# typio/entreepy

Measured on AMD Instinct MI355X. Metric: GB/s encode+decode on 1 GiB text at 1/2/4/8 MI355X; % of HBM read peak, higher is better.
Workload: dtype u8; 1 GPU; text-1G: 1073741824 B per GPU, order-0 samples of a_midsummer_nights_dream.txt's byte distribution, seed 0x5EED0004+rank, one step = encode to .et + decode back, HBM-resident; bytes_per_gpu=1073741824, packed_bytes_per_gpu=629699194

## Files before the change

entreepy_amd/codec.py:

```python
import ctypes
from dataclasses import dataclass

import numpy as np

from . import _native as N


class EntreepyError(RuntimeError):
    def __init__(self, status, detail=""):
        msg = N.lib().et_strerror(status).decode()
        super().__init__(f"{msg}{': ' + detail if detail else ''} (et_status {status})")
        self.status = status


class EmptyInputError(EntreepyError):
    """The reference's error.QueueEmpty (queue.zig:28-30 reached from encode.zig:137-138)."""


@dataclass
class EncodeFlags:
    write_output: bool = False
    print_output: bool = False
    debug: bool = False

# ... 150 lines not shown
        _check(N.lib().et_ctx_reserve(self._h, int(max_text_bytes)), self._h)

    def set_tile_rounds(self, rounds):
        _check(N.lib().et_ctx_set_tile_rounds(self._h, int(rounds)), self._h)

    TIMING_DECODE_BODY = 2

    def enable_timing(self, on=True):
        _check(N.lib().et_ctx_enable_timing(self._h, 2 if (on is not True and on == self.TIMING_DECODE_BODY) else int(bool(on))), self._h)

    def timings(self, which=None):
        t = N.Timings()
        if which is None:
            _check(N.lib().et_last_timings(self._h, ctypes.byref(t)), self._h)
        else:
            _check(N.lib().et_last_timings_of(self._h, {"encode": 0, "decode": 1}[which], ctypes.byref(t)), self._h)
        d = {k: getattr(t, k) for k, _ in N.Timings._fields_ if k not in ("reserved", "pad_")}
        d["exhaustive_sync"] = bool(t.reserved & 1)
        d["tree_walk_sync"] = bool(t.reserved & 2)
        d["chained_write"] = bool(t.reserved & 4)
        d["row_sync"] = bool(t.reserved & 8)
        d["fixed_sync"] = bool(t.reserved & 16)
        d["strips_write"] = bool(t.reserved & 32)
        return d

    def last_codebook(self):
        cb = Codebook()
        _check(N.lib().et_last_codebook(self._h, ctypes.byref(cb.raw)), self._h)
        return cb

    def encode_file(self, in_path, out_path=None):
        return self._file_call(N.lib().et_encode_fd, in_path, out_path, ())

    def decode_file(self, in_path, out_path=None, skip=4):
        return self._file_call(N.lib().et_decode_fd, in_path, out_path, (skip,))

    def _file_call(self, fn, in_path, out_path, extra):
        import os

        fin = os.open(in_path, os.O_RDONLY)
        fout = os.open(out_path, os.O_RDWR | os.O_CREAT | os.O_TRUNC, 0o644) if out_path is not None else -1
        try:
            a, b = ctypes.c_size_t(0), ctypes.c_size_t(0)
            _check(fn(self._h, fin, *extra, fout, ctypes.byref(a), ctypes.byref(b)), self._h)
            return a.value, b.value
        finally:
# ... 371 lines not shown
```

entreepy_amd/csrc/et_api.cpp:

```cpp
#include <sys/stat.h>

#include "et_ctx.h"

#include <algorithm>
#include <cstdlib>
#include <vector>

namespace {

struct Geometry {
    const uint8_t *base;
    uint64_t lo, hi;
    uint32_t rpt, n_tiles;
};

Geometry make_geometry(const et_ctx *ctx, const void *d_text, size_t n) {
    Geometry g;
    const uintptr_t a = reinterpret_cast<uintptr_t>(d_text);
    g.base = reinterpret_cast<const uint8_t *>(a & ~static_cast<uintptr_t>(15));
    g.lo = a & 15;
    g.hi = g.lo + n;
    uint32_t rpt = 1;
    while (rpt < et::MAX_ROUNDS_PER_TILE && g.hi / (static_cast<uint64_t>(rpt) * et::ROUND_BYTES) > 2048) rpt <<= 1;
    if (ctx && ctx->force_rpt) rpt = ctx->force_rpt;
// ... 34 lines not shown
    ctx->hist_tiles = g.n_tiles;
    ctx->hist_on_host = false;
    return ET_OK;
}

int run_body(et_ctx *ctx, const et_codebook *cb, const Geometry &g, uint32_t *out32, uint64_t base_bit,
             const uint8_t *header, size_t header_len, int ev_scan, int ev_body) {
    const bool long_codes = cb->max_length > 32;
    ET_TRY(wait_for_word<uint64_t>(ctx, ctx->h_scalar + HS_ENC_TAKEN, ctx->enc_block_epoch, 100.0, "the code table block was never taken"));
    for (int s = 0; s < 256; ++s) {
        const uint32_t len = cb->length[s];
        uint32_t code = cb->data[s];
        if (!long_codes) code = len ? (len == 32 ? code : (code & ((1u << len) - 1u)) << (32 - len)) : 0u;
        ctx->h_enc[2 * s] = code;
        ctx->h_enc[2 * s + 1] = len;
        ctx->h_enc[512 + s] = len;
    }
    const size_t padded = (header_len + 3) & ~static_cast<size_t>(3);
    if (header_len) {
        if (padded > HEADER_STAGE) return fail(ctx, ET_ERR_ARG, "header too long");
        uint8_t *stage = reinterpret_cast<uint8_t *>(ctx->h_enc + 768);
        std::memcpy(stage, header, header_len);
        std::memset(stage + header_len, 0, padded - header_len);
    }
    et::launch_tile_scan(ctx->stream, static_cast<const uint32_t *>(ctx->tile_hist.p), g.n_tiles, cb->length, ctx->h_enc, static_cast<uint32_t *>(ctx->enc_table.p),
                         static_cast<uint32_t>(768 + padded / 4), reinterpret_cast<unsigned long long *>(ctx->h_scalar + HS_ENC_TAKEN), ++ctx->enc_block_epoch,
                         static_cast<unsigned long long *>(ctx->tile_bits.p),
                         static_cast<unsigned long long *>(ctx->group_sum.p), scan_epoch(ctx), base_bit,
                         static_cast<unsigned long long *>(ctx->tile_off.p), out32, static_cast<const uint32_t *>(ctx->enc_table.p) + 768,
                         static_cast<uint32_t>(padded / 4));
    ET_HIP(hipGetLastError());
    et::launch_encode(ctx->stream, g.base, g.lo, g.hi, g.rpt, g.n_tiles, static_cast<const unsigned long long *>(ctx->tile_off.p),
                      static_cast<const uint2 *>(ctx->enc_table.p), cb->max_length, out32, timed(ctx, ev_scan, ev_body));
    ET_HIP(hipGetLastError());
    return ET_OK;
}

int fetch_histogram(et_ctx *ctx) {
    if (ctx->hist_on_host) return ET_OK;
    for (uint32_t w = 0; w < et::HIST_REDUCE_GROUPS; ++w)
        ET_TRY(wait_for_word<uint64_t>(ctx, ctx->h_hist + 256 + w, ctx->hist_epoch, 100.0, "the histogram never reached the host"));
    ctx->hist_on_host = true;
    return ET_OK;
}

}
// ... 24 lines not shown
    ok = ok && hipHostMalloc(reinterpret_cast<void **>(&ctx->h_enc), 768 * sizeof(uint32_t) + HEADER_STAGE) == hipSuccess;
    ok = ok && hipHostMalloc(reinterpret_cast<void **>(&ctx->h_header), HEADER_STAGE) == hipSuccess;
    for (int i = 0; i < 2; ++i) ok = ok && hipHostMalloc(reinterpret_cast<void **>(&ctx->h_lut_buf[i]), DEC_TABLES_BYTES) == hipSuccess;
    ok = ok && hipHostMalloc(reinterpret_cast<void **>(&ctx->h_scalar), HS_SLOTS * sizeof(uint64_t)) == hipSuccess;
    if (ok) std::memset(ctx->h_scalar, 0, HS_SLOTS * sizeof(uint64_t));
    for (int i = 0; i < 2; ++i) ok = ok && hipHostMalloc(reinterpret_cast<void **>(&ctx->h_tw_tree[i]), sizeof(et::TwUpload)) == hipSuccess;
    for (auto &e : ctx->ev) ok = ok && hipEventCreateWithFlags(&e, hipEventDisableSystemFence) == hipSuccess;
    if (!ok) {
        et_ctx_destroy(ctx);
        return ET_ERR_HIP;
    }
    *out = ctx;
    return ET_OK;
}

extern "C" void et_ctx_destroy(et_ctx *ctx) {
    if (!ctx) return;
    DeviceGuard guard(ctx->device);
    (void)hipStreamSynchronize(ctx->stream);
    DevBuf *bufs[] = {&ctx->tile_hist, &ctx->block_hist, &ctx->hist, &ctx->tile_bits, &ctx->tile_off, &ctx->enc_table, &ctx->group_sum,
                      &ctx->sub_state, &ctx->blk_exit, &ctx->blk_count, &ctx->blk_off, &ctx->lut, &ctx->flag,
                      &ctx->worklist, &ctx->lane_maps, &ctx->blk_maps, &ctx->grp_maps, &ctx->blk_in, &ctx->grp_in, &ctx->row_scratch,
                      &ctx->tw_table, &ctx->tw_tree, &ctx->blk_start, &ctx->blk_pub, &ctx->chain_table, &ctx->io_in, &ctx->io_out,
                      &ctx->batch_jobs, &ctx->batch_blob, &ctx->batch_counter};
    for (DevBuf *b : bufs)
        if (b->p) (void)hipFree(b->p);
    delete ctx->io;
    void *pinned[] = {ctx->h_hist, ctx->h_enc, ctx->h_header, ctx->h_lut_buf[0], ctx->h_lut_buf[1], ctx->h_scalar, ctx->h_tw_tree[0], ctx->h_tw_tree[1], ctx->h_batch};
    for (void *p : pinned)
        if (p) (void)hipHostFree(p);
    for (auto &e : ctx->ev)
        if (e) (void)hipEventDestroy(e);
    if (ctx->own_stream) (void)hipStreamDestroy(ctx->own_stream);
    if (ctx->side.stream) (void)hipStreamDestroy(ctx->side.stream);
    if (ctx->side.fork) (void)hipEventDestroy(ctx->side.fork);
    if (ctx->side.join) (void)hipEventDestroy(ctx->side.join);
    if (ctx->switch_ev) (void)hipEventDestroy(ctx->switch_ev);
    delete ctx;
}

namespace {

int switch_stream(et_ctx *ctx, hipStream_t s) {
    if (s == ctx->stream) return ET_OK;
    DeviceGuard guard(ctx->device);
    ET_HIP(hipEventRecord(ctx->switch_ev, ctx->stream));
    ET_HIP(hipStreamWaitEvent(s, ctx->switch_ev, 0));
// ... 40 lines not shown
        ET_HIP(hipEventSynchronize(ctx->ev[3]));
        if (!ctx->pend_enc_shard) {
            ctx->tm_enc.hist_ms = elapsed(ctx, 0, 1);
            ctx->tm_enc.total_ms = elapsed(ctx, 0, 3);
        }
        ctx->tm_enc.scan_ms = ctx->pend_enc_bits ? elapsed(ctx, 1, 2) : 0.f;
        ctx->tm_enc.body_ms = elapsed(ctx, 2, 3);
        ctx->pend_enc = ctx->pend_enc_shard = false;
    }
    if (which == 1 && ctx->pend_dec && ctx->timing_body) {
        ET_HIP(hipEventSynchronize(ctx->ev[EV_DEC + 3]));
        ctx->tm_dec.body_ms = elapsed(ctx, EV_DEC + 2, EV_DEC + 3);
        ctx->pend_dec = false;
    }
    if (which == 1 && ctx->pend_dec) {
        ET_HIP(hipEventSynchronize(ctx->ev[EV_DEC + 3]));
        ctx->tm_dec.sync_ms = elapsed(ctx, EV_DEC + 0, EV_DEC + 2);
        ctx->tm_dec.scan_ms = elapsed(ctx, EV_DEC + 5, EV_DEC + 2);
        ctx->tm_dec.body_ms = elapsed(ctx, EV_DEC + 2, EV_DEC + 3);
        ctx->tm_dec.total_ms = elapsed(ctx, EV_DEC + 0, EV_DEC + 3);
        ctx->tm_dec.sync_first_ms = ctx->pend_dec_first ? elapsed(ctx, EV_DEC + 0, EV_DEC + 5) : 0.f;
        ctx->pend_dec = false;
    }
    *out = which == 0 ? ctx->tm_enc : ctx->tm_dec;
    return ET_OK;
}

extern "C" int et_last_timings(et_ctx *ctx, et_timings *out) {
    if (!ctx) return ET_ERR_ARG;
    return et_last_timings_of(ctx, ctx->last_kind, out);
}

extern "C" int et_last_codebook(const et_ctx *ctx, et_codebook *out) {
    if (!ctx || !out) return ET_ERR_ARG;
    if (!ctx->have_cb) return ET_ERR_ARG;
    *out = ctx->last_cb;
    return ET_OK;
}

extern "C" int et_ctx_reserve(et_ctx *ctx, size_t max_text_bytes) {
    if (!ctx) return ET_ERR_ARG;
    DeviceGuard guard(ctx->device);
    const Geometry g = make_geometry(nullptr, reinterpret_cast<const void *>(static_cast<uintptr_t>(15)), max_text_bytes);
    ET_TRY(ensure_encode_ws(ctx, g.n_tiles + 1));
    const uint64_t n_subs = (static_cast<uint64_t>(max_text_bytes) + 8192) * 8 / et::SUB_BITS + 2;
    const uint64_t n_blocks = n_subs / et::BLOCK + 2;
// ... 25 lines not shown
        return ET_OK;
    }
    ctx->hist_empty = false;
    const Geometry g = make_geometry(ctx, d_text, n);
    ET_TRY(run_histogram(ctx, d_text, n, g, d_hist));
    if (ctx->timing) {
        ET_HIP(hipStreamSynchronize(ctx->stream));
        ctx->tm_enc = et_timings{};
        ctx->tm_enc.hist_ms = elapsed(ctx, 0, 1);
        ctx->pend_enc = false;
        ctx->last_kind = 0;
    }
    return ET_OK;
}

namespace {

int encode_shard(et_ctx *ctx, const et_codebook *cb, const void *d_text, size_t n, void *d_out, size_t cap_bytes, uint64_t start_bit,
                 const uint8_t *header, size_t header_len, uint64_t *end_bit) {
    if (!ctx || !cb || !d_out || !end_bit || (n && !d_text)) return ET_ERR_ARG;
    if (reinterpret_cast<uintptr_t>(d_out) & 3) return fail(ctx, ET_ERR_ARG, "d_out must be 4-byte aligned");
    if (header_len > HEADER_STAGE - 4) return fail(ctx, ET_ERR_ARG, "header too long");
    DeviceGuard guard(ctx->device);
    auto empty_shard = [&]() -> int {
        const size_t head_words = (header_len + 3) / 4;
        const size_t own_word = header_len ? 0 : static_cast<size_t>(start_bit / 32);
        const size_t need = (header_len ? head_words : own_word + 1) * 4;
        if (need > cap_bytes) return fail(ctx, ET_ERR_CAP, "body does not fit d_out");
        if (header_len) {
            std::memset(ctx->h_header, 0, head_words * 4);
            std::memcpy(ctx->h_header, header, header_len);
            ET_HIP(hipMemcpyAsync(d_out, ctx->h_header, head_words * 4, hipMemcpyHostToDevice, ctx->stream));
        } else {
            ET_HIP(hipMemsetAsync(static_cast<uint8_t *>(d_out) + own_word * 4, 0, 4, ctx->stream));
        }
        *end_bit = start_bit;
        return ET_OK;
    };
    if (n == 0) {
        ET_HIP(hipStreamSynchronize(ctx->stream));
        return empty_shard();
    }
    if (ctx->hist_text != d_text || ctx->hist_n != n)
        return fail(ctx, ET_ERR_ARG, "shard encode needs et_histogram_device on the same (d_text, n) first");
    ET_TRY(fetch_histogram(ctx));
    ET_HIP(hipStreamSynchronize(ctx->stream));
// ... 48 lines not shown
    std::memcpy(ctx->h_hist, counts, 256 * sizeof(uint64_t));
    ctx->hist_on_host = true;
    return ET_OK;
}

extern "C" int et_encode_body_device(et_ctx *ctx, const et_codebook *cb, const void *d_text, size_t n, void *d_out, size_t cap_bytes,
                                     uint64_t start_bit, uint64_t *end_bit) {
    return encode_shard(ctx, cb, d_text, n, d_out, cap_bytes, start_bit, nullptr, 0, end_bit);
}

extern "C" int et_encode_head_shard_device(et_ctx *ctx, const et_codebook *cb, const void *d_text, size_t n, void *d_out, size_t cap_bytes,
                                           const uint8_t *header, size_t header_len, uint64_t *end_bit) {
    if (!header || !header_len) return ET_ERR_ARG;
    return encode_shard(ctx, cb, d_text, n, d_out, cap_bytes, static_cast<uint64_t>(header_len) * 8, header, header_len, end_bit);
}

extern "C" int et_encode_device(et_ctx *ctx, const void *d_text, size_t n, void *d_out, size_t cap, size_t *out_len) {
    if (!ctx || !d_out || !out_len || (n && !d_text)) return ET_ERR_ARG;
    *out_len = 0;
    if (n == 0) return fail(ctx, ET_ERR_EMPTY, "empty input");
    if (reinterpret_cast<uintptr_t>(d_out) & 15) return fail(ctx, ET_ERR_ARG, "d_out must be 16-byte aligned");
    if (cap < et_encode_bound(n)) return fail(ctx, ET_ERR_CAP, "cap < et_encode_bound(n)");
    DeviceGuard guard(ctx->device);
    const Geometry g = make_geometry(ctx, d_text, n);
    ET_TRY(run_histogram(ctx, d_text, n, g));
    ET_TRY(fetch_histogram(ctx));
    const double t1 = now_ms();

    et_codebook cb;
    int rc = et_build_codebook(ctx->h_hist, &cb);
    if (rc != ET_OK) return fail(ctx, rc, "et_build_codebook");
    ctx->last_cb = cb;
    ctx->have_cb = true;
    size_t header_len = 0;
    std::memset(ctx->h_header, 0, HEADER_STAGE);
    rc = et_write_header(&cb, n, ctx->h_header, HEADER_STAGE - 4, &header_len);
    if (rc != ET_OK) return fail(ctx, rc, "et_write_header");
    uint64_t bits = 0;
    et_codebook_bits(&cb, ctx->h_hist, &bits);
    const double t2 = now_ms();

    if (bits == 0) {
        const size_t padded = (header_len + 3) & ~static_cast<size_t>(3);
        ET_HIP(hipMemcpyAsync(d_out, ctx->h_header, padded, hipMemcpyHostToDevice, ctx->stream));
        record(ctx, 2);
        record(ctx, 3);
// ... 167 lines not shown
```

entreepy_amd/csrc/et_ctx.h:

```cpp
#pragma once

#include "entreepy_hip.h"

#include "et_io.h"
#include "et_kernels.h"
#include "et_rowsync.h"
#include "et_tables.h"
#include "et_treewalk.h"

#include <hip/hip_runtime.h>

#include <atomic>
#include <chrono>
#include <cstdio>
#include <cstring>
#include <string>

struct DevBuf {
    void *p = nullptr;
    size_t cap = 0;
};

constexpr size_t HEADER_STAGE = 8192;
constexpr size_t DEC_TABLES_BYTES = et::DecTableLayout::BYTES;

enum class Family { TREE_WALK, WINDOWS, ROWS, FIXED_SYNC, FIXED_WRITE, EXIT_MAPS };

using et::DecWs;

struct Span : et::DecSpan {
    uint32_t tw_mode, dec_flags, row_mode;
    const et_codebook *cb;
    et::RowCode row_code;
    et::DecodeTables tb, tb_write;
    const uint16_t *tw_table;
    uint32_t tw_n_int;
    uint32_t *blk_start, *blk_pub;
    uint32_t *exit_bits;
    const uint64_t *chain;
    uint32_t n_chain;
};

enum HostScalar {
    HS_TOTAL = 1,
    HS_RANGE_FLAGS = 2,
    HS_BODY_FLAGS = 4,
    HS_ENC_TAKEN = 12,
    HS_HEADER_DONE = 14,
    HS_SLOTS = 16
};
enum RangeFlag { RF_START = 0, RF_EXIT = 1, RF_ROW_BLIND = 2 };

struct et_ctx {
    int device = 0;
    hipStream_t own_stream = nullptr;
    et::SideLane side = {};
    hipStream_t stream = nullptr;
    hipEvent_t switch_ev = nullptr;
    bool timing = false;
    bool timing_body = false;
    uint32_t force_rpt = 0;
    std::string err;

    DevBuf tile_hist, block_hist, hist, tile_bits, tile_off, enc_table, group_sum;
    DevBuf sub_state, blk_exit, blk_count, blk_off, lut, flag, worklist;
    DevBuf lane_maps, blk_maps, grp_maps, blk_in, grp_in;
    DevBuf row_scratch;
    DevBuf tw_table, tw_tree, blk_start, blk_pub, chain_table;
    et::TwUpload *h_tw_tree[2] = {};
    int tw_turn = 0;
    DevBuf io_in, io_out;
    et_io::Pipe *io = nullptr;

    DevBuf batch_jobs, batch_blob, batch_counter;
    uint8_t *h_batch = nullptr;
    uint64_t batch_epoch = 0;

    uint64_t *h_hist = nullptr;
    uint32_t *h_enc = nullptr;
    uint8_t *h_header = nullptr;
    uint8_t *h_lut_buf[2] = {};
    int lut_turn = 0;
    uint64_t *h_scalar = nullptr;

    const void *hist_text = nullptr;
    size_t hist_n = 0;
    uint32_t hist_rpt = 0, hist_tiles = 0;
// ... 68 lines not shown
        b.p = nullptr;
        return fail(ctx, e == hipErrorOutOfMemory ? ET_ERR_NOMEM : ET_ERR_HIP, "hipMalloc", e);
    }
    b.cap = want;
    return ET_OK;
}

#define ET_TRY(expr)                 \
    do {                             \
        int rc_ = (expr);            \
        if (rc_ != ET_OK) return rc_; \
    } while (0)

inline uint32_t scan_epoch(et_ctx *ctx) {
    if (ctx->group_sum.p != ctx->scan_buf || ctx->group_sum.cap != ctx->scan_cap || ctx->scan_epoch_n >= 0xffffu) {
        (void)hipMemsetAsync(ctx->group_sum.p, 0, ctx->group_sum.cap, ctx->stream);
        ctx->scan_buf = ctx->group_sum.p;
        ctx->scan_cap = ctx->group_sum.cap;
        ctx->scan_epoch_n = 0;
    }
    return ++ctx->scan_epoch_n;
}

inline void record(et_ctx *ctx, int i) {
    if (ctx->timing) (void)hipEventRecord(ctx->ev[i], ctx->stream);
}

constexpr int EV_DEC = 6;

inline et::KernelEvents timed(et_ctx *ctx, int a, int b) { return ctx->timing ? et::KernelEvents{ctx->ev[a], ctx->ev[b]} : et::KernelEvents{}; }

inline et::KernelEvents timed_body(et_ctx *ctx, int a, int b) {
    return ctx->timing || ctx->timing_body ? et::KernelEvents{ctx->ev[a], ctx->ev[b]} : et::KernelEvents{};
}

inline double now_ms() {
    return std::chrono::duration<double, std::milli>(std::chrono::steady_clock::now().time_since_epoch()).count();
}

template <typename T>
int wait_for_word(et_ctx *ctx, volatile const T *word, T want, double patience_ms, const char *what) {
    const double t0 = now_ms();
    for (uint32_t spin = 0; *word != want; ++spin)
        if ((spin & 1023u) == 1023u && now_ms() - t0 > patience_ms) {
            ET_HIP(hipStreamSynchronize(ctx->stream));
            if (*word != want) return fail(ctx, ET_ERR_HIP, what);
        }
    std::atomic_thread_fence(std::memory_order_acquire);
    return ET_OK;
}
```

entreepy_amd/csrc/et_kernels.h:

```cpp
#pragma once

#include <hip/hip_runtime.h>
#include <stdint.h>

#include "et_tables.h"

#ifdef ET_GUARD_DROP_PINS
#define ET_PIN(x_) ((void)0)
#else
#define ET_PIN(x_) asm volatile("" : "+v"(x_))
#endif

namespace et {

constexpr int BLOCK = 256;
constexpr uint32_t ROUND_BYTES = BLOCK * 16;
constexpr uint32_t MAX_ROUNDS_PER_TILE = 128;
constexpr uint32_t HIST_REDUCE_GROUPS = 128;
constexpr uint32_t MAX_GRID = 2048;

constexpr uint32_t SUB_BITS = 256;
constexpr uint32_t DEC_BLOCK_WORDS = BLOCK * SUB_BITS / 32;
constexpr uint32_t DEC_GUARD_WORDS = 4;
constexpr uint32_t SYNC_CHUNK = 1, WRITE_CHUNK = 4;
// ... 42 lines not shown
    uint32_t n_blocks, first_bit;
};

struct SideLane {
    hipStream_t stream;
    hipEvent_t fork, join;
};

struct KernelEvents {
    hipEvent_t start = nullptr, stop = nullptr;
};

void launch_hist(hipStream_t stream, const uint8_t *base, uint64_t lo, uint64_t hi, uint32_t rounds_per_tile, uint32_t n_tiles,
                 uint32_t *tile_hist, unsigned long long *block_hist, unsigned long long *hist, unsigned long long *host_hist = nullptr, unsigned long long epoch = 0,
                 KernelEvents ev = {}, unsigned long long *hist_also = nullptr);
__host__ __device__ inline uint32_t header_bound(uint8_t d) { return 8u + 6u * (static_cast<uint32_t>(d) + 1u); }
void launch_words_to_host(hipStream_t stream, const void *d_src, uint32_t n_words, void *host_dst, unsigned long long *host_done, unsigned long long epoch);
void launch_header_to_host(hipStream_t stream, const void *d_src, uint32_t n, void *host_dst, unsigned long long *host_done, unsigned long long epoch);
void launch_tile_scan(hipStream_t stream, const uint32_t *tile_hist, uint32_t n_tiles, const uint8_t *lengths, const uint32_t *host_src, uint32_t *dev_dst,
                      uint32_t copy_words, unsigned long long *host_taken, unsigned long long taken_epoch, unsigned long long *tile_bits, unsigned long long *group_sum, uint32_t epoch, unsigned long long base_bit,
                      unsigned long long *tile_off, uint32_t *out32, const uint32_t *header_src = nullptr, uint32_t header_words = 0);
void launch_encode(hipStream_t stream, const uint8_t *base, uint64_t lo, uint64_t hi, uint32_t rounds_per_tile, uint32_t n_tiles,
                   const unsigned long long *tile_off, const uint2 *enc_table, uint32_t max_len, uint32_t *out32, KernelEvents ev = {});
void launch_dec_sync(hipStream_t stream, const DecSpan &s, const DecodeTables &tb, uint32_t iter, uint32_t max_trips, uint32_t flags = DEC_HAVE_START,
                     bool listed = false, const SideLane *side = nullptr, bool ticket_is_zero = false, KernelEvents ev = {});
void launch_dec_maps(hipStream_t stream, const DecSpan &s, bool have_start, const DecodeTables &tb, uint32_t n_starts, uint32_t map_stride,
                     uint8_t *lane_maps, uint8_t *blk_maps, uint8_t *grp_maps);
void launch_dec_resolve(hipStream_t stream, const DecSpan &s, bool const_first, const DecodeTables &tb, uint32_t map_stride, const uint8_t *lane_maps,
                        const uint8_t *blk_maps, const uint8_t *grp_maps, uint8_t *blk_in, uint8_t *grp_in);
void launch_build_dec_tables(hipStream_t stream, uint8_t *d_block, size_t wsteps_at, size_t plan_at, uint32_t *zero16 = nullptr);
struct ScanVerify { const uint32_t *state; bool rows; uint32_t first; };
struct ScanReport { uint32_t *host; uint32_t epoch; };
void launch_dec_scan(hipStream_t stream, const DecSpan &s, uint32_t epoch, const ScanVerify *verify = nullptr, const ScanReport *report = nullptr);
void launch_dec_write(hipStream_t stream, const DecSpan &s, const DecodeTables &tb, uint64_t n_symbols, uint8_t *out, DecFlag ticket = FLAG_SYNC_TICKET,
                      const SideLane *side = nullptr, bool ticket_is_zero = false, bool speculative = false, KernelEvents ev = {},
                      const uint64_t *chain = nullptr, uint32_t n_chain = 0, uint32_t chain_max_len = 32, bool strips = false);

}
```

entreepy_amd/csrc/et_kernels.hip:

```cpp
#include "et_kernels_common.h"
#include "et_treewalk.h"

namespace et {

#ifndef ET_NT_LOAD_K1
#define ET_NT_LOAD_K1 1
#endif
#ifndef ET_NT_LOAD_K4
#define ET_NT_LOAD_K4 0
#endif
#ifndef ET_NT_STORE_K4
#define ET_NT_STORE_K4 0
#endif

struct Chunk {
    uint32_t w[4];
    uint32_t valid;
};

__device__ __forceinline__ Chunk load_chunk(const uint8_t *__restrict__ base, uint64_t off, uint64_t lo, uint64_t hi) {
    Chunk c;
    if (off >= lo && off + 16 <= hi) {
        const uint4 v = *reinterpret_cast<const uint4 *>(base + off);
        c.w[0] = v.x; c.w[1] = v.y; c.w[2] = v.z; c.w[3] = v.w;
// ... 255 lines not shown
        const unsigned long long total = prefix + group_total;
        out[n] = total;
        if (total_copy) *total_copy = total;
        if (zero_words && (total >> 5) != seam && (total & 31)) zero_words[total >> 5] = 0;
        if (report_dst) {
            for (int k = 0; k < 12; ++k) report_dst[k] = report_src[k];
            if (verify_state) report_dst[2] = (bad_before || bad_any) ? 1u : 0u;
            report_dst[12] = static_cast<uint32_t>(total);
            report_dst[13] = static_cast<uint32_t>(total >> 32);
            pinned_stores_visible();
            __hip_atomic_store(report_dst + 14, report_epoch, __ATOMIC_RELEASE, __HIP_MEMORY_SCOPE_SYSTEM);
        }
    }
    if (g == 0 && header_words) {
        __syncthreads();
        for (uint32_t k = tid; k < header_words; k += 1024) zero_words[k] = header_src[k];
    }
}

struct RingFlush {
    uint32_t *ring;
    uint32_t *out32;
    bool first_word_shared;
};

template <uint32_t RING_WORDS>
__device__ __forceinline__ void flush_words(const RingFlush &f, uint32_t from, uint32_t to) {
    for (uint32_t i = from + threadIdx.x; i < to; i += BLOCK) {
        const uint32_t slot = i & (RING_WORDS - 1);
        const uint32_t v = __builtin_bswap32(f.ring[slot]);
        f.ring[slot] = 0;
        if (i == 0 && f.first_word_shared) atomicOr(f.out32, v);
#if ET_NT_STORE_K4
        else __builtin_nontemporal_store(v, f.out32 + i);
#else
        else f.out32[i] = v;
#endif
    }
}

template <uint32_t RING_WORDS>
__global__ __launch_bounds__(BLOCK) void k_encode_tiles(const uint8_t *__restrict__ base, uint64_t lo, uint64_t hi,
                                                        uint32_t rounds_per_tile, uint32_t n_tiles,
                                                        const unsigned long long *__restrict__ tile_off,
                                                        const uint2 *__restrict__ enc_table, uint32_t *__restrict__ out32) {
    __shared__ __attribute__((aligned(16))) uint32_t ring[RING_WORDS];
    __shared__ __attribute__((aligned(16))) uint2 tab[256];
    __shared__ uint32_t scratch[2][4];
    const int tid = threadIdx.x;
    tab[tid] = enc_table[tid];
    for (uint32_t i = tid; i < RING_WORDS; i += BLOCK) ring[i] = 0;
    __syncthreads();

    const uint64_t tile_bytes = static_cast<uint64_t>(rounds_per_tile) * ROUND_BYTES;
    for (uint32_t t = blockIdx.x; t < n_tiles; t += gridDim.x) {
        const unsigned long long bit0 = tile_off[t];
        RingFlush f;
        f.ring = ring;
        f.out32 = out32 + (bit0 >> 5);
        f.first_word_shared = (bit0 & 31) != 0;
        uint32_t run = static_cast<uint32_t>(bit0 & 31);
        uint32_t flushed = 0;
        const uint64_t t0 = static_cast<uint64_t>(t) * tile_bytes + static_cast<uint64_t>(tid) * 16;
        const bool interior = static_cast<uint64_t>(t) * tile_bytes >= lo && static_cast<uint64_t>(t + 1) * tile_bytes <= hi;

        Chunk cur = load_chunk_in_tile<ET_NT_LOAD_K4>(base, t0, lo, hi, interior);
#pragma unroll
        for (int k = 0; k < 4; ++k) ET_PIN(cur.w[k]);
        for (uint32_t r = 0; r < rounds_per_tile; ++r) {
            Chunk nxt;
            nxt.valid = 0;
            nxt.w[0] = nxt.w[1] = nxt.w[2] = nxt.w[3] = 0;
            if (r + 1 < rounds_per_tile) nxt = load_chunk_in_tile<ET_NT_LOAD_K4>(base, t0 + static_cast<uint64_t>(r + 1) * ROUND_BYTES, lo, hi, interior);

#define ET_ENTRY(k_) tab[(cur.w[(k_) >> 2] >> (8 * ((k_) & 3))) & 0xffu]
            uint32_t qcode[4], qlen[4];
            uint32_t tot = 0;
            bool wide4 = false;
            if (cur.valid == 0xffffu) {
#pragma unroll
                for (int q = 0; q < 4; ++q) {
                    const uint2 e0 = ET_ENTRY(4 * q), e1 = ET_ENTRY(4 * q + 1), e2 = ET_ENTRY(4 * q + 2), e3 = ET_ENTRY(4 * q + 3);
                    const uint32_t l01 = e0.y + e1.y, l23 = e2.y + e3.y;
// ... 49 lines not shown
                        if (__builtin_amdgcn_ballot_w64(qlen[q] > 32) == 0) {
                            ET_APPEND(qcode[q], qlen[q]);
                        } else {
                            const uint2 e0 = ET_ENTRY(4 * q), e1 = ET_ENTRY(4 * q + 1), e2 = ET_ENTRY(4 * q + 2), e3 = ET_ENTRY(4 * q + 3);
                            ET_APPEND(e0.x | (e1.x >> (e0.y & 31u)), e0.y + e1.y);
                            ET_APPEND(e2.x | (e3.x >> (e2.y & 31u)), e2.y + e3.y);
                        }
                    }
                } else {
                    for (int k = 0; k < 16; ++k) {
                        uint2 e = ET_ENTRY(k);
                        if (!((cur.valid >> k) & 1u)) e = make_uint2(0u, 0u);
                        ET_APPEND(e.x, e.y);
                    }
                }
            }
#undef ET_APPEND
#undef ET_ENTRY
            if (fill) atomicOr(reinterpret_cast<uint32_t *>(ring_bytes + wbyte), part);
            run += round_total;
            __syncthreads();
#pragma unroll
            for (int k = 0; k < 4; ++k) ET_PIN(nxt.w[k]);
            flush_words<RING_WORDS>(f, flushed, run >> 5);
            flushed = run >> 5;
            cur = nxt;
        }
        if ((run & 31) && tid == 0) {
            const uint32_t slot = flushed & (RING_WORDS - 1);
            atomicOr(f.out32 + flushed, __builtin_bswap32(ring[slot]));
            ring[slot] = 0;
        }
        __syncthreads();
    }
}

__global__ __launch_bounds__(BLOCK) void k_encode_tiles_long(const uint8_t *__restrict__ base, uint64_t lo, uint64_t hi,
                                                             uint32_t rounds_per_tile, uint32_t n_tiles,
                                                             const unsigned long long *__restrict__ tile_off,
                                                             const uint2 *__restrict__ enc_table, uint32_t *__restrict__ out32) {
    constexpr uint32_t RING_WORDS = 4096;
    __shared__ uint32_t ring[RING_WORDS];
    __shared__ uint2 tab[256];
    __shared__ uint32_t scratch[2][4];
    const int tid = threadIdx.x;
    tab[tid] = enc_table[tid];
    for (uint32_t i = tid; i < RING_WORDS; i += BLOCK) ring[i] = 0;
    __syncthreads();

    const uint64_t tile_bytes = static_cast<uint64_t>(rounds_per_tile) * ROUND_BYTES;
    const uint32_t steps = rounds_per_tile * (ROUND_BYTES / BLOCK);
// ... 372 lines not shown
    hipLaunchKernelGGL(k_words_to_host, dim3(1), dim3(1024), 0, stream, static_cast<const uint32_t *>(d_src), n_words, static_cast<uint32_t *>(host_dst), host_done, epoch);
}

void launch_header_to_host(hipStream_t stream, const void *d_src, uint32_t n, void *host_dst, unsigned long long *host_done, unsigned long long epoch) {
    hipLaunchKernelGGL(k_header_to_host, dim3(1), dim3(1024), 0, stream, static_cast<const uint8_t *>(d_src), n, static_cast<uint32_t *>(host_dst), host_done, epoch);
}

void launch_tile_scan(hipStream_t stream, const uint32_t *tile_hist, uint32_t n_tiles, const uint8_t *lengths, const uint32_t *host_src, uint32_t *dev_dst,
                      uint32_t copy_words, unsigned long long *host_taken, unsigned long long taken_epoch, unsigned long long *tile_bits, unsigned long long *group_sum, uint32_t epoch, unsigned long long base_bit,
                      unsigned long long *tile_off, uint32_t *out32, const uint32_t *header_src, uint32_t header_words) {
    uint32_t grid = (n_tiles + 3) / 4;
    if (grid > MAX_GRID) grid = MAX_GRID;
    CodeLengths cl;
    for (int l = 0; l < 64; ++l) cl.packed[l] = lengths[4 * l] | (lengths[4 * l + 1] << 8) | (lengths[4 * l + 2] << 16) | (static_cast<uint32_t>(lengths[4 * l + 3]) << 24);
    hipLaunchKernelGGL(k_tile_bits, dim3(grid), dim3(BLOCK), 0, stream, tile_hist, n_tiles, cl, tile_bits, host_src, dev_dst, copy_words, host_taken, taken_epoch);
    const uint32_t groups = (n_tiles + 1023) / 1024;
    hipLaunchKernelGGL(k_scan_fused<unsigned long long>, dim3(groups), dim3(1024), 0, stream, tile_bits, n_tiles, tile_off, group_sum, epoch, base_bit, out32, header_src,
                       header_words, static_cast<unsigned long long *>(nullptr), static_cast<const uint32_t *>(nullptr), static_cast<const uint32_t *>(nullptr),
                       static_cast<uint32_t *>(nullptr), 0xffffffffu, 0u, 0u, static_cast<const uint32_t *>(nullptr), static_cast<uint32_t *>(nullptr), 0u);
}

void launch_encode(hipStream_t stream, const uint8_t *base, uint64_t lo, uint64_t hi, uint32_t rounds_per_tile, uint32_t n_tiles,
                   const unsigned long long *tile_off, const uint2 *enc_table, uint32_t max_len, uint32_t *out32, KernelEvents ev) {
    if (max_len > 32)
        ET_LAUNCH_TIMED(k_encode_tiles_long, dim3(tile_grid(k_encode_tiles_long, n_tiles)), dim3(BLOCK), 0, stream, ev, base, lo, hi, rounds_per_tile, n_tiles, tile_off, enc_table, out32);
    else if (max_len <= 31)
        ET_LAUNCH_TIMED(k_encode_tiles<4096>, dim3(tile_grid(k_encode_tiles<4096>, n_tiles)), dim3(BLOCK), 0, stream, ev, base, lo, hi, rounds_per_tile, n_tiles, tile_off, enc_table, out32);
    else
        ET_LAUNCH_TIMED(k_encode_tiles<8192>, dim3(tile_grid(k_encode_tiles<8192>, n_tiles)), dim3(BLOCK), 0, stream, ev, base, lo, hi, rounds_per_tile, n_tiles, tile_off, enc_table, out32);
}

void launch_dec_scan(hipStream_t stream, const DecSpan &s, uint32_t epoch, const ScanVerify *verify, const ScanReport *report) {
    const uint32_t groups = (s.n_blocks + 1023) / 1024;
    const bool rows = verify && verify->rows;
    hipLaunchKernelGGL(k_scan_fused<uint32_t>, dim3(groups), dim3(1024), 0, stream, static_cast<const uint32_t *>(s.blk_count), s.n_blocks, s.blk_off, s.group_sum, epoch, 0ull,
                       static_cast<uint32_t *>(nullptr), static_cast<const uint32_t *>(nullptr), 0u,
                       report ? reinterpret_cast<unsigned long long *>(s.flag + FLAG_TOTAL_LO) : nullptr, verify ? verify->state : nullptr,
                       verify ? static_cast<const uint32_t *>(s.blk_exit) : nullptr, verify ? s.flag + FLAG_VERIFY_FAILED : nullptr, verify ? verify->first : 0xffffffffu,
                       rows ? 1u : static_cast<uint32_t>(BLOCK), rows ? 0xffffffffu : 0xffu, report ? static_cast<const uint32_t *>(s.flag) : nullptr,
                       report ? report->host : nullptr, report ? report->epoch : 0u);
}

void launch_dec_write(hipStream_t stream, const DecSpan &s, const DecodeTables &tb, uint64_t n_symbols, uint8_t *out, DecFlag ticket, const SideLane *side,
                      bool ticket_is_zero, bool speculative, KernelEvents ev, const uint64_t *chain, uint32_t n_chain, uint32_t chain_max_len, bool strips) {
    const uint32_t *words = s.words, *sub_state = s.sub_state, *void_flags = speculative ? s.flag : nullptr;
    if (chain) {
        constexpr int WAVES = 8;
        const size_t smem_wave = ((static_cast<size_t>(n_chain) * 8 + 15) & ~static_cast<size_t>(15)) + WAVES * WV_STAGE_ALLOC;
        const uint32_t n_units = (s.n_blocks * 4 + WAVES - 1) / WAVES;
        if (strips) {
            const size_t smem_strips = ((static_cast<size_t>(n_chain) * 8 + 15) & ~static_cast<size_t>(15)) + WAVES * WS_ALLOC;
            ET_LAUNCH_TIMED((k_dec_write_wave<WAVES, true>), dim3(decode_grid(k_dec_write_wave<WAVES, true>, smem_strips, n_units, true, 64 * WAVES)), dim3(64 * WAVES), smem_strips, stream, ev, words, s.n_bytes, s.n_blocks, reinterpret_cast<const uint2 *>(chain), n_chain, sub_state, s.blk_off, n_symbols, out, void_flags, s.n_subs, chain_max_len);
// ... 11 lines not shown
```

include/entreepy_hip.h:

```cpp
#ifndef ENTREEPY_HIP_H
#define ENTREEPY_HIP_H

#include <stddef.h>
#include <stdint.h>

#ifdef __cplusplus
extern "C" {
#endif

typedef enum et_status {
    ET_OK = 0,
    ET_ERR_EMPTY = 1,
    ET_ERR_NOMEM = 2,
    ET_ERR_CAP = 3,
    ET_ERR_FORMAT = 4,
    ET_ERR_HIP = 5,
    ET_ERR_ARG = 6,
    ET_ERR_UNSUPPORTED = 7,
    ET_ERR_IO = 8,
    ET_ERR_RCCL = 9
} et_status;

typedef struct et_codebook {
    uint32_t data[256];
    uint8_t length[256];
    uint8_t dfs_order[256];
    uint32_t n_coded;
    uint32_t min_length;
    uint32_t max_length;
} et_codebook;

typedef struct et_timings {
    float hist_ms;
    float host_ms;
    float scan_ms;
    float body_ms;
    float sync_ms;
    float total_ms;
    uint32_t sync_iters;
    uint32_t reserved;
    float sync_first_ms;
    uint32_t pad_;
} et_timings;

typedef struct et_ctx et_ctx;

int et_ctx_create(int device, et_ctx **ctx);
void et_ctx_destroy(et_ctx *ctx);
int et_ctx_set_stream(et_ctx *ctx, void *hip_stream);
int et_ctx_use_own_stream(et_ctx *ctx);
void *et_ctx_stream(const et_ctx *ctx);
int et_ctx_device(const et_ctx *ctx);
int et_ctx_reserve(et_ctx *ctx, size_t max_text_bytes);
int et_ctx_set_tile_rounds(et_ctx *ctx, uint32_t rounds);
#define ET_TIMING_DECODE_BODY 2
int et_ctx_enable_timing(et_ctx *ctx, int on);
int et_last_timings(et_ctx *ctx, et_timings *out);
int et_last_timings_of(et_ctx *ctx, int which, et_timings *out);
const char *et_last_error(const et_ctx *ctx);
const char *et_strerror(int status);
const char *et_version(void);

size_t et_encode_bound(size_t text_len);

int et_encode(et_ctx *ctx, const uint8_t *text, size_t n,
              uint8_t *out, size_t cap, size_t *out_len);
// ... 142 lines not shown
```

Measured before the change: 889.6 GB/s.

## Fuse encode tile-offset scan and table upload into the encode kernel via decoupled lookback

When every tile fits in one resident workgroup, the encode kernel now computes each tile's bit count from its histogram, publishes it, and derives its starting bit offset through a two-level lookback (groups of 32 tiles) in place of a separate scan kernel. Workgroup 0 copies the code table from pinned host memory into replicated device slots that the other workgroups poll, and boundary words between tiles are stitched through published tails instead of atomicOr. This removes a kernel launch and the tile_off round trip. In exchange it relies on all workgroups being co-resident, adds spin-waits with a fault path on timeout, and serialises the tile tail stitching.

```diff
diff --git a/entreepy_amd/codec.py b/entreepy_amd/codec.py
--- a/entreepy_amd/codec.py
+++ b/entreepy_amd/codec.py
@@ -196,6 +196,7 @@
         d["row_sync"] = bool(t.reserved & 8)
         d["fixed_sync"] = bool(t.reserved & 16)
         d["strips_write"] = bool(t.reserved & 32)
+        d["reserved"] = int(t.reserved)
         return d
 
     def last_codebook(self):
diff --git a/entreepy_amd/csrc/et_api.cpp b/entreepy_amd/csrc/et_api.cpp
--- a/entreepy_amd/csrc/et_api.cpp
+++ b/entreepy_amd/csrc/et_api.cpp
@@ -80,6 +80,26 @@
         uint8_t *stage = reinterpret_cast<uint8_t *>(ctx->h_enc + 768);
         std::memcpy(stage, header, header_len);
         std::memset(stage + header_len, 0, padded - header_len);
+    }
+    ctx->enc_self = et::encode_self_scan_fits(g.n_tiles, cb->max_length);
+    if (ctx->enc_self) {
+        et::SelfScan ss = {};
+        ET_TRY(self_epoch(ctx, &ss.epoch));
+        ss.tile_hist = static_cast<const uint32_t *>(ctx->tile_hist.p);
+        ss.tile_pub = static_cast<unsigned long long *>(ctx->self_words.p);
+        ss.tile_tail = ss.tile_pub + et::MAX_GRID;
+        ss.tile_grp = ss.tile_tail + et::MAX_GRID;
+        ss.table = ss.tile_grp + et::MAX_GRID / et::SELF_GROUP;
+        ss.host_src = ctx->h_enc;
+        ss.host_taken = reinterpret_cast<unsigned long long *>(ctx->h_scalar + HS_ENC_TAKEN);
+        ss.host_fault = reinterpret_cast<unsigned long long *>(ctx->h_scalar + HS_ENC_FAULT);
+        ss.taken_epoch = ++ctx->enc_block_epoch;
+        ss.base_bit = base_bit;
+        ss.tag = static_cast<uint32_t>(ss.taken_epoch % 0xfffffeull) + 1u;
+        ss.header_words = static_cast<uint32_t>(padded / 4);
+        et::launch_encode_self(ctx->stream, g.base, g.lo, g.hi, g.rpt, g.n_tiles, cb->length, ss, cb->max_length, out32, timed(ctx, ev_scan, ev_body));
+        ET_HIP(hipGetLastError());
+        return ET_OK;
     }
     et::launch_tile_scan(ctx->stream, static_cast<const uint32_t *>(ctx->tile_hist.p), g.n_tiles, cb->length, ctx->h_enc, static_cast<uint32_t *>(ctx->enc_table.p),
                          static_cast<uint32_t>(768 + padded / 4), reinterpret_cast<unsigned long long *>(ctx->h_scalar + HS_ENC_TAKEN), ++ctx->enc_block_epoch,
@@ -150,7 +170,7 @@
                       &ctx->sub_state, &ctx->blk_exit, &ctx->blk_count, &ctx->blk_off, &ctx->lut, &ctx->flag,
                       &ctx->worklist, &ctx->lane_maps, &ctx->blk_maps, &ctx->grp_maps, &ctx->blk_in, &ctx->grp_in, &ctx->row_scratch,
                       &ctx->tw_table, &ctx->tw_tree, &ctx->blk_start, &ctx->blk_pub, &ctx->chain_table, &ctx->io_in, &ctx->io_out,
-                      &ctx->batch_jobs, &ctx->batch_blob, &ctx->batch_counter};
+                      &ctx->batch_jobs, &ctx->batch_blob, &ctx->batch_counter, &ctx->self_words};
     for (DevBuf *b : bufs)
         if (b->p) (void)hipFree(b->p);
     delete ctx->io;
@@ -237,6 +257,7 @@
         ctx->tm_dec.sync_first_ms = ctx->pend_dec_first ? elapsed(ctx, EV_DEC + 0, EV_DEC + 5) : 0.f;
         ctx->pend_dec = false;
     }
+    if (which == 0) ctx->tm_enc.reserved = ctx->enc_self ? ET_TM_ENC_SELF_SCAN : 0u;
     *out = which == 0 ? ctx->tm_enc : ctx->tm_dec;
     return ET_OK;
 }
@@ -308,6 +329,7 @@
     if (reinterpret_cast<uintptr_t>(d_out) & 3) return fail(ctx, ET_ERR_ARG, "d_out must be 4-byte aligned");
     if (header_len > HEADER_STAGE - 4) return fail(ctx, ET_ERR_ARG, "header too long");
     DeviceGuard guard(ctx->device);
+    ctx->enc_self = false;
     auto empty_shard = [&]() -> int {
         const size_t head_words = (header_len + 3) / 4;
         const size_t own_word = header_len ? 0 : static_cast<size_t>(start_bit / 32);
@@ -402,6 +424,7 @@
     if (reinterpret_cast<uintptr_t>(d_out) & 15) return fail(ctx, ET_ERR_ARG, "d_out must be 16-byte aligned");
     if (cap < et_encode_bound(n)) return fail(ctx, ET_ERR_CAP, "cap < et_encode_bound(n)");
     DeviceGuard guard(ctx->device);
+    ctx->enc_self = false;
     const Geometry g = make_geometry(ctx, d_text, n);
     ET_TRY(run_histogram(ctx, d_text, n, g));
     ET_TRY(fetch_histogram(ctx));
diff --git a/entreepy_amd/csrc/et_ctx.h b/entreepy_amd/csrc/et_ctx.h
--- a/entreepy_amd/csrc/et_ctx.h
+++ b/entreepy_amd/csrc/et_ctx.h
@@ -46,6 +46,7 @@
     HS_RANGE_FLAGS = 2,
     HS_BODY_FLAGS = 4,
     HS_ENC_TAKEN = 12,
+    HS_ENC_FAULT = 13,
     HS_HEADER_DONE = 14,
     HS_SLOTS = 16
 };
@@ -63,6 +64,9 @@
     std::string err;
 
     DevBuf tile_hist, block_hist, hist, tile_bits, tile_off, enc_table, group_sum;
+    DevBuf self_words;
+    uint32_t self_epoch_n = 0;
+    bool enc_self = false;
     DevBuf sub_state, blk_exit, blk_count, blk_off, lut, flag, worklist;
     DevBuf lane_maps, blk_maps, grp_maps, blk_in, grp_in;
     DevBuf row_scratch;
@@ -177,6 +181,17 @@
     return ++ctx->scan_epoch_n;
 }
 
+inline int self_epoch(et_ctx *ctx, uint32_t *epoch) {
+    const bool fresh = ctx->self_words.p == nullptr;
+    ET_TRY(ensure(ctx, ctx->self_words, et::SELF_WORDS * sizeof(uint64_t)));
+    if (fresh || ctx->self_epoch_n >= 0xffffu) {
+        ET_HIP(hipMemsetAsync(ctx->self_words.p, 0, ctx->self_words.cap, ctx->stream));
+        ctx->self_epoch_n = 0;
+    }
+    *epoch = ++ctx->self_epoch_n;
+    return ET_OK;
+}
+
 inline void record(et_ctx *ctx, int i) {
     if (ctx->timing) (void)hipEventRecord(ctx->ev[i], ctx->stream);
 }
@@ -202,5 +217,9 @@
             if (*word != want) return fail(ctx, ET_ERR_HIP, what);
         }
     std::atomic_thread_fence(std::memory_order_acquire);
+    if (*reinterpret_cast<volatile const uint64_t *>(ctx->h_scalar + HS_ENC_FAULT) != 0) {
+        ctx->h_scalar[HS_ENC_FAULT] = 0;
+        return fail(ctx, ET_ERR_HIP, "an encode workgroup gave up waiting for the tiles before it; the image of that encode is incomplete");
+    }
     return ET_OK;
 }
diff --git a/entreepy_amd/csrc/et_kernels.h b/entreepy_amd/csrc/et_kernels.h
--- a/entreepy_amd/csrc/et_kernels.h
+++ b/entreepy_amd/csrc/et_kernels.h
@@ -88,6 +88,25 @@
                       unsigned long long *tile_off, uint32_t *out32, const uint32_t *header_src = nullptr, uint32_t header_words = 0);
 void launch_encode(hipStream_t stream, const uint8_t *base, uint64_t lo, uint64_t hi, uint32_t rounds_per_tile, uint32_t n_tiles,
                    const unsigned long long *tile_off, const uint2 *enc_table, uint32_t max_len, uint32_t *out32, KernelEvents ev = {});
+constexpr uint32_t SELF_GROUP = 32;
+constexpr uint32_t SELF_REPLICAS = 16;
+constexpr uint32_t SELF_REPLICA_STRIDE = 512;
+constexpr size_t SELF_WORDS = 2 * static_cast<size_t>(MAX_GRID) + MAX_GRID / SELF_GROUP + static_cast<size_t>(SELF_REPLICAS) * SELF_REPLICA_STRIDE;
+struct SelfScan {
+    const uint32_t *tile_hist;
+    unsigned long long *tile_pub;
+    unsigned long long *tile_grp;
+    unsigned long long *tile_tail;
+    unsigned long long *table;
+    const uint32_t *host_src;
+    unsigned long long *host_taken;
+    unsigned long long *host_fault;
+    unsigned long long taken_epoch, base_bit;
+    uint32_t epoch, tag, header_words;
+};
+bool encode_self_scan_fits(uint32_t n_tiles, uint32_t max_len);
+void launch_encode_self(hipStream_t stream, const uint8_t *base, uint64_t lo, uint64_t hi, uint32_t rounds_per_tile, uint32_t n_tiles, const uint8_t *lengths,
+                        const SelfScan &ss, uint32_t max_len, uint32_t *out32, KernelEvents ev = {});
 void launch_dec_sync(hipStream_t stream, const DecSpan &s, const DecodeTables &tb, uint32_t iter, uint32_t max_trips, uint32_t flags = DEC_HAVE_START,
                      bool listed = false, const SideLane *side = nullptr, bool ticket_is_zero = false, KernelEvents ev = {});
 void launch_dec_maps(hipStream_t stream, const DecSpan &s, bool have_start, const DecodeTables &tb, uint32_t n_starts, uint32_t map_stride,
diff --git a/entreepy_amd/csrc/et_kernels.hip b/entreepy_amd/csrc/et_kernels.hip
--- a/entreepy_amd/csrc/et_kernels.hip
+++ b/entreepy_amd/csrc/et_kernels.hip
@@ -301,15 +301,19 @@
     uint32_t *ring;
     uint32_t *out32;
     bool first_word_shared;
+    uint32_t *first_word;
 };
 
-template <uint32_t RING_WORDS>
+template <uint32_t RING_WORDS, bool SELF = false>
 __device__ __forceinline__ void flush_words(const RingFlush &f, uint32_t from, uint32_t to) {
     for (uint32_t i = from + threadIdx.x; i < to; i += BLOCK) {
         const uint32_t slot = i & (RING_WORDS - 1);
         const uint32_t v = __builtin_bswap32(f.ring[slot]);
         f.ring[slot] = 0;
-        if (i == 0 && f.first_word_shared) atomicOr(f.out32, v);
+        if (i == 0 && f.first_word_shared) {
+            if (SELF) *f.first_word = v;
+            else atomicOr(f.out32, v);
+        }
 #if ET_NT_STORE_K4
         else __builtin_nontemporal_store(v, f.out32 + i);
 #else
@@ -318,26 +322,112 @@
     }
 }
 
-template <uint32_t RING_WORDS>
+constexpr uint32_t SELF_POLLS = 1u << 20;
+constexpr unsigned long long SELF_BITS_MASK = (1ull << 48) - 1ull;
+static_assert(MAX_GRID / SELF_GROUP <= 64 && SELF_GROUP <= 64, "one wavefront reads the group sums, and a group's totals");
+
+__device__ __forceinline__ bool self_wait(const unsigned long long *word, uint32_t shift, uint32_t want, unsigned long long *v) {
+    for (uint32_t poll = 0; poll < SELF_POLLS; ++poll) {
+        *v = __hip_atomic_load(word, __ATOMIC_RELAXED, __HIP_MEMORY_SCOPE_AGENT);
+        if ((*v >> shift) == want) return true;
+        __builtin_amdgcn_s_sleep(8);
+    }
+    return false;
+}
+
+template <uint32_t RING_WORDS, bool SELF = false>
 __global__ __launch_bounds__(BLOCK) void k_encode_tiles(const uint8_t *__restrict__ base, uint64_t lo, uint64_t hi,
                                                         uint32_t rounds_per_tile, uint32_t n_tiles,
                                                         const unsigned long long *__restrict__ tile_off,
-                                                        const uint2 *__restrict__ enc_table, uint32_t *__restrict__ out32) {
+                                                        const uint2 *__restrict__ enc_table, uint32_t *__restrict__ out32,
+                                                        const SelfScan ss, const CodeLengths lengths) {
     __shared__ __attribute__((aligned(16))) uint32_t ring[RING_WORDS];
     __shared__ __attribute__((aligned(16))) uint2 tab[256];
     __shared__ uint32_t scratch[2][4];
+    __shared__ unsigned long long self_sum[1];
+    __shared__ uint32_t self_word[3];
     const int tid = threadIdx.x;
-    tab[tid] = enc_table[tid];
-    for (uint32_t i = tid; i < RING_WORDS; i += BLOCK) ring[i] = 0;
-    __syncthreads();
+    unsigned long long self_bit0 = 0;
+    if (SELF) {
+        const uint32_t t = blockIdx.x, lane = tid & 63;
+        if (tid == 0) self_word[0] = self_word[1] = self_word[2] = 0;
+        for (uint32_t i = tid; i < RING_WORDS; i += BLOCK) ring[i] = 0;
+        __syncthreads();
+        bool seen = true;
+        const unsigned long long tag48 = static_cast<unsigned long long>(ss.epoch) << 48;
+        if (tid < 64) {
+            const uint32_t l4 = lengths.packed[lane];
+            const uint4 c = reinterpret_cast<const uint4 *>(ss.tile_hist + static_cast<uint64_t>(t) * 256)[lane];
+            unsigned long long s = static_cast<unsigned long long>(c.x) * (l4 & 0xffu) + static_cast<unsigned long long>(c.y) * ((l4 >> 8) & 0xffu) +
+                                   static_cast<unsigned long long>(c.z) * ((l4 >> 16) & 0xffu) + static_cast<unsigned long long>(c.w) * (l4 >> 24);
+#pragma unroll
+            for (int d = 32; d >= 1; d >>= 1) s += __shfl_xor(s, d, 64);
+            if (lane == 0) __hip_atomic_store(ss.tile_pub + t, tag48 | s, __ATOMIC_RELAXED, __HIP_MEMORY_SCOPE_AGENT);
+            const uint32_t g0 = t & ~(SELF_GROUP - 1);
+            unsigned long long mine = 0;
+            if (lane < SELF_GROUP && g0 + lane < t) {
+                seen = self_wait(ss.tile_pub + g0 + lane, 48, ss.epoch, &mine);
+                mine &= SELF_BITS_MASK;
+            }
+            unsigned long long before = mine;
+#pragma unroll
+            for (int d = 32; d >= 1; d >>= 1) before += __shfl_xor(before, d, 64);
+            const bool group_seen = __all(seen);
+            if ((t & (SELF_GROUP - 1)) == SELF_GROUP - 1 && lane == 0 && group_seen)
+                __hip_atomic_store(ss.tile_grp + t / SELF_GROUP, tag48 | (before + s), __ATOMIC_RELAXED, __HIP_MEMORY_SCOPE_AGENT);
+            unsigned long long grp = 0;
+            if (lane < t / SELF_GROUP) {
+                seen = self_wait(ss.tile_grp + lane, 48, ss.epoch, &grp) && seen;
+                grp &= SELF_BITS_MASK;
+            }
+#pragma unroll
+            for (int d = 32; d >= 1; d >>= 1) grp += __shfl_xor(grp, d, 64);
+            if (lane == 0) self_sum[0] = before + grp;
+        }
+        if (t == 0) {
+            const uint2 e = reinterpret_cast<const uint2 *>(ss.host_src)[tid];
+            const uint32_t whole = static_cast<uint32_t>(ss.base_bit >> 5) < ss.header_words ? static_cast<uint32_t>(ss.base_bit >> 5) : ss.header_words;
+            if (tid == 0 && whole < ss.header_words) self_word[1] = __builtin_bswap32(ss.host_src[768 + whole]);
+            const unsigned long long entry = static_cast<unsigned long long>(ss.tag) << 40 | static_cast<unsigned long long>(e.y & 0xffu) << 32 | e.x;
+#pragma unroll
+            for (uint32_t r = 0; r < SELF_REPLICAS; ++r) __hip_atomic_store(ss.table + r * SELF_REPLICA_STRIDE + tid, entry, __ATOMIC_RELAXED, __HIP_MEMORY_SCOPE_AGENT);
+            tab[tid] = make_uint2(e.x, e.y & 0xffu);
+            for (uint32_t i0 = tid; i0 < whole; i0 += 8 * BLOCK) {
+                uint32_t v[8];
+#pragma unroll
+                for (int k = 0; k < 8; ++k) v[k] = i0 + k * BLOCK < whole ? ss.host_src[768 + i0 + k * BLOCK] : 0u;
+#pragma unroll
+                for (int k = 0; k < 8; ++k)
+                    if (i0 + k * BLOCK < whole) out32[i0 + k * BLOCK] = v[k];
+            }
+        } else {
+            unsigned long long v;
+            seen = self_wait(ss.table + (t & (SELF_REPLICAS - 1)) * SELF_REPLICA_STRIDE + tid, 40, ss.tag, &v) && seen;
+            tab[tid] = make_uint2(static_cast<uint32_t>(v), static_cast<uint32_t>(v >> 32) & 0xffu);
+        }
+        if (!seen) self_word[2] = 1;
+        __syncthreads();
+        if (t == 0) {
+            if (tid == 0) __hip_atomic_store(ss.host_taken, ss.taken_epoch, __ATOMIC_RELAXED, __HIP_MEMORY_SCOPE_SYSTEM);
+        } else if (self_word[2]) {
+            if (tid == 0) __hip_atomic_store(ss.host_fault, ss.taken_epoch, __ATOMIC_RELAXED, __HIP_MEMORY_SCOPE_SYSTEM);
+            return;
+        }
+        self_bit0 = ss.base_bit + self_sum[0];
+    } else {
+        tab[tid] = enc_table[tid];
+        for (uint32_t i = tid; i < RING_WORDS; i += BLOCK) ring[i] = 0;
+        __syncthreads();
+    }
 
     const uint64_t tile_bytes = static_cast<uint64_t>(rounds_per_tile) * ROUND_BYTES;
     for (uint32_t t = blockIdx.x; t < n_tiles; t += gridDim.x) {
-        const unsigned long long bit0 = tile_off[t];
+        const unsigned long long bit0 = SELF ? self_bit0 : tile_off[t];
         RingFlush f;
         f.ring = ring;
         f.out32 = out32 + (bit0 >> 5);
         f.first_word_shared = (bit0 & 31) != 0;
+        f.first_word = self_word;
         uint32_t run = static_cast<uint32_t>(bit0 & 31);
         uint32_t flushed = 0;
         const uint64_t t0 = static_cast<uint64_t>(t) * tile_bytes + static_cast<uint64_t>(tid) * 16;
@@ -433,11 +523,32 @@
             __syncthreads();
 #pragma unroll
             for (int k = 0; k < 4; ++k) ET_PIN(nxt.w[k]);
-            flush_words<RING_WORDS>(f, flushed, run >> 5);
+            flush_words<RING_WORDS, SELF>(f, flushed, run >> 5);
             flushed = run >> 5;
             cur = nxt;
         }
-        if ((run & 31) && tid == 0) {
+        if (SELF) {
+            if (tid == 0) {
+                const uint32_t slot = flushed & (RING_WORDS - 1);
+                uint32_t tail = (run & 31) ? ring[slot] : 0u;
+                ring[slot] = 0;
+                bool seen = true;
+                if (f.first_word_shared) {
+                    unsigned long long before = self_word[1];
+                    if (t > 0) seen = self_wait(ss.tile_tail + (t - 1), 48, ss.epoch, &before);
+                    const uint32_t pred = static_cast<uint32_t>(before);
+                    if (flushed && seen) f.out32[0] = self_word[0] | __builtin_bswap32(pred);
+                    else tail |= pred;
+                }
+                if (!seen) __hip_atomic_store(ss.host_fault, ss.taken_epoch, __ATOMIC_RELAXED, __HIP_MEMORY_SCOPE_SYSTEM);
+                else if (t + 1 == n_tiles) {
+                    if (run & 31) f.out32[flushed] = __builtin_bswap32(tail);
+                } else {
+                    __hip_atomic_store(ss.tile_tail + t, static_cast<unsigned long long>(ss.epoch) << 48 | static_cast<unsigned long long>(run & 31) << 32 | tail, __ATOMIC_RELAXED,
+                                       __HIP_MEMORY_SCOPE_AGENT);
+                }
+            }
+        } else if ((run & 31) && tid == 0) {
             const uint32_t slot = flushed & (RING_WORDS - 1);
             atomicOr(f.out32 + flushed, __builtin_bswap32(ring[slot]));
             ring[slot] = 0;
@@ -856,12 +967,31 @@
 
 void launch_encode(hipStream_t stream, const uint8_t *base, uint64_t lo, uint64_t hi, uint32_t rounds_per_tile, uint32_t n_tiles,
                    const unsigned long long *tile_off, const uint2 *enc_table, uint32_t max_len, uint32_t *out32, KernelEvents ev) {
+    const SelfScan none = {};
+    const CodeLengths no_lengths = {};
     if (max_len > 32)
         ET_LAUNCH_TIMED(k_encode_tiles_long, dim3(tile_grid(k_encode_tiles_long, n_tiles)), dim3(BLOCK), 0, stream, ev, base, lo, hi, rounds_per_tile, n_tiles, tile_off, enc_table, out32);
     else if (max_len <= 31)
-        ET_LAUNCH_TIMED(k_encode_tiles<4096>, dim3(tile_grid(k_encode_tiles<4096>, n_tiles)), dim3(BLOCK), 0, stream, ev, base, lo, hi, rounds_per_tile, n_tiles, tile_off, enc_table, out32);
+        ET_LAUNCH_TIMED(k_encode_tiles<4096>, dim3(tile_grid(k_encode_tiles<4096>, n_tiles)), dim3(BLOCK), 0, stream, ev, base, lo, hi, rounds_per_tile, n_tiles, tile_off, enc_table, out32, none, no_lengths);
     else
-        ET_LAUNCH_TIMED(k_encode_tiles<8192>, dim3(tile_grid(k_encode_tiles<8192>, n_tiles)), dim3(BLOCK), 0, stream, ev, base, lo, hi, rounds_per_tile, n_tiles, tile_off, enc_table, out32);
+        ET_LAUNCH_TIMED(k_encode_tiles<8192>, dim3(tile_grid(k_encode_tiles<8192>, n_tiles)), dim3(BLOCK), 0, stream, ev, base, lo, hi, rounds_per_tile, n_tiles, tile_off, enc_table, out32, none, no_lengths);
+}
+
+bool encode_self_scan_fits(uint32_t n_tiles, uint32_t max_len) {
+    if (max_len > 32 || n_tiles == 0) return false;
+    return max_len <= 31 ? tile_grid(k_encode_tiles<4096, true>, n_tiles) == n_tiles : tile_grid(k_encode_tiles<8192, true>, n_tiles) == n_tiles;
+}
+
+void launch_encode_self(hipStream_t stream, const uint8_t *base, uint64_t lo, uint64_t hi, uint32_t rounds_per_tile, uint32_t n_tiles, const uint8_t *lengths,
+                        const SelfScan &ss, uint32_t max_len, uint32_t *out32, KernelEvents ev) {
+    CodeLengths cl;
+    for (int l = 0; l < 64; ++l) cl.packed[l] = lengths[4 * l] | (lengths[4 * l + 1] << 8) | (lengths[4 * l + 2] << 16) | (static_cast<uint32_t>(lengths[4 * l + 3]) << 24);
+    const unsigned long long *no_off = nullptr;
+    const uint2 *no_table = nullptr;
+    if (max_len <= 31)
+        ET_LAUNCH_TIMED((k_encode_tiles<4096, true>), dim3(n_tiles), dim3(BLOCK), 0, stream, ev, base, lo, hi, rounds_per_tile, n_tiles, no_off, no_table, out32, ss, cl);
+    else
+        ET_LAUNCH_TIMED((k_encode_tiles<8192, true>), dim3(n_tiles), dim3(BLOCK), 0, stream, ev, base, lo, hi, rounds_per_tile, n_tiles, no_off, no_table, out32, ss, cl);
 }
 
 void launch_dec_scan(hipStream_t stream, const DecSpan &s, uint32_t epoch, const ScanVerify *verify, const ScanReport *report) {
diff --git a/include/entreepy_hip.h b/include/entreepy_hip.h
--- a/include/entreepy_hip.h
+++ b/include/entreepy_hip.h
@@ -42,6 +42,8 @@
     float sync_first_ms;
     uint32_t pad_;
 } et_timings;
+
+#define ET_TM_ENC_SELF_SCAN 1u
 
 typedef struct et_ctx et_ctx;
 
```

Result: slower. 844.6 GB/s (-5.1%).
